# kch3782/torcwa

Measured on AMD Instinct MI355X. Metric: RCWA layer-solves/sec (complex64 I/O) at Fourier order [15,15], higher is better.
Workload: dtype c128 results (mixed-precision eigensolver: fp32 eigendecomposition refined to fp64 by two Newton steps -- fp64 residual and update GEMMs, the correction solved with ONE fp32 LU of the fp32 start; everything else fp64 MFMA); complex64 I/O; 1 GPU; configs[1]: single patterned layer, order=[15,15] (n=1922), 300x300 grid, 128-lambda sweep, glass input half-space; points_total=128, points_per_gpu=128, layer_solves_per_point=1, chunk=128, streams=1, precision=high

## Files before the change

torcwa_amd/csrc/eig_qr.hip:

```cpp
#include "eig.hpp"
#include <cstdlib>
#include <limits>
#include <mutex>
#include <string>
#include <thread>
#include <vector>
#include "mfma.hpp"
#include "prof.hpp"

namespace trx {
namespace {

constexpr int QW = EigPlan::QW, QNS = EigPlan::QNS, QKC = EigPlan::QKC;
constexpr int SM = 64;
constexpr int QAED = EigPlan::QAED;
constexpr int QAED_MOVES = 12;

template <class T>
struct Rot {
    T c;
    cx<T> s, r;
};

template <class T>
// ... 31 lines not shown
        if (!(big < std::numeric_limits<T>::infinity())) { R.c = T(1); R.s = cx<T>(T(0), T(0)); R.r = f; return R; }
        int ex;
        (void)frexp((double)big, &ex);
        const T sc = (T)ldexp(1.0, -ex), isc = (T)ldexp(1.0, ex);
        const cx<T> fs = sc * f, gs = sc * g;
        const T a2 = norm2(fs), g2 = norm2(gs), m2 = a2 + g2;
        if (a2 == T(0)) { const T ng = sqrt(g2); R.c = T(0); R.s = (T(1) / ng) * conj(gs); R.r = cx<T>(ng * isc, T(0)); return R; }
        const T t2 = T(1) / sqrt(a2 * m2);
        R.c = a2 * t2;
        R.s = t2 * (fs * conj(gs));
        R.r = ((m2 * t2) * isc) * fs;
    }
    return R;
}

template <class T, bool BC = false>
__device__ bool small_schur(cx<T>* Hs, int m, cx<T>* Us, Rot<T>* rots, const int SLD, long long* dbg = nullptr, int* nrot_out = nullptr) {
    const auto sync = [] { __syncthreads(); };
    const int lane = threadIdx.x;
    long long t_left = 0, t_right = 0, t_u = 0, t_pre = 0, tt = 0, n_it = 0, n_rot = 0;
    if (dbg) tt = clock64();
    const T ulp = eps_of<T>::value;
    int ihi = m - 1, its = 0, total = 0, nrot = 0;
    while (ihi > 0) {
        int small = 0;
        if (lane >= 1 && lane <= ihi) {
            const cx<T> sub = Hs[lane * SLD + lane - 1];
            T sc = abs1(Hs[(lane - 1) * SLD + lane - 1]) + abs1(Hs[lane * SLD + lane]);
            if (sc == T(0)) sc = T(1);
            small = (abs1(sub) <= ulp * sc);
            if (small) Hs[lane * SLD + lane - 1] = cx<T>(T(0), T(0));
        }
        const unsigned long long mask = __ballot(small);
        const int l = mask ? (63 - __builtin_clzll(mask)) : 0;
        sync();
        if (l == ihi) { --ihi; its = 0; continue; }
        ++its; ++total;
        if (total > 40 * m) { if (nrot_out) *nrot_out = nrot; return false; }
        nrot += ihi - l;
        cx<T> sig;
        {
            const cx<T> a = Hs[(ihi - 1) * SLD + ihi - 1], bq = Hs[(ihi - 1) * SLD + ihi], cq = Hs[ihi * SLD + ihi - 1], d = Hs[ihi * SLD + ihi];
            if (its % 10 == 0) {
                sig = d + cx<T>(T(0.75) * fabs(cq.x), T(0));
            } else {
                const cx<T> tr = T(0.5) * (a + d);
                const cx<T> det = (a - tr) * (d - tr) - bq * cq;
                const cx<T> sq = csqrt(-det);
                const cx<T> e1 = tr + sq, e2 = tr - sq;
                sig = (abs1(e1 - d) < abs1(e2 - d)) ? e1 : e2;
            }
        }
        sync();
        if (lane >= l && lane <= ihi) Hs[lane * SLD + lane] -= sig;
        sync();
        if (dbg) { const long long t1 = clock64(); t_pre += t1 - tt; tt = t1; n_it += 1; n_rot += ihi - l; }
        {
            const bool mine = (lane >= l && lane < m);
            cx<T> xcur = mine ? Hs[l * SLD + lane] : cx<T>(T(0), T(0));
            cx<T> ynext = (mine && l + 1 <= ihi) ? Hs[(l + 1) * SLD + lane] : cx<T>(T(0), T(0));
            for (int r = l; r < ihi; ++r) {
                const cx<T> ypre = (mine && r + 2 <= ihi) ? Hs[(r + 2) * SLD + lane] : cx<T>(T(0), T(0));
                Rot<T> R;
                if constexpr (BC) {
                    R = rotg_fast(bcast_lane(xcur, r), bcast_lane(ynext, r));
                } else {
                    R.c = T(1); R.s = cx<T>(T(0), T(0)); R.r = cx<T>(T(0), T(0));
                    if (lane == r) R = rotg_fast(xcur, ynext);
                    R.c = __shfl(R.c, r);
                    R.s.x = __shfl(R.s.x, r); R.s.y = __shfl(R.s.y, r);
                    R.r.x = __shfl(R.r.x, r); R.r.y = __shfl(R.r.y, r);
                }
                if (lane == r) rots[r] = R;
                if (lane >= r && lane < m) {
                    cx<T> x = xcur, y = ynext;
                    rot_rows(R, x, y);
                    if (lane == r) { x = R.r; y = cx<T>(T(0), T(0)); Hs[(r + 1) * SLD + lane] = y; }
                    Hs[r * SLD + lane] = x;
                    xcur = y;
                }
                ynext = ypre;
            }
            if (lane >= ihi && lane < m) Hs[ihi * SLD + lane] = xcur;
        }
        sync();
        if (dbg) { const long long t1 = clock64(); t_left += t1 - tt; tt = t1; }
        {
        if (lane <= ihi) {
            const int i = lane;
            const int r0 = (i - 1 > l) ? i - 1 : l;
            if (r0 < ihi) {
                cx<T> x = Hs[i * SLD + r0];
                for (int r = r0; r < ihi; ++r) {
                    cx<T> y = Hs[i * SLD + r + 1];
                    rot_cols(rots[r], x, y);
                    Hs[i * SLD + r] = x;
                    x = y;
                }
                Hs[i * SLD + ihi] = x;
            }
        }
        if (dbg) { sync(); const long long t1 = clock64(); t_right += t1 - tt; tt = t1; }
        if (Us && lane < m && l < ihi) {
            cx<T> x = Us[lane * SLD + l];
            for (int r = l; r < ihi; ++r) {
                cx<T> y = Us[lane * SLD + r + 1];
                rot_cols(rots[r], x, y);
                Us[lane * SLD + r] = x;
                x = y;
            }
            Us[lane * SLD + ihi] = x;
        }
        sync();
        if (dbg) { const long long t1 = clock64(); t_u += t1 - tt; tt = t1; }
        }
        if (lane >= l && lane <= ihi) Hs[lane * SLD + lane] += sig;
        sync();
    }
    if (dbg && lane == 0) { dbg[0] += t_pre; dbg[1] += t_left; dbg[2] += t_right; dbg[3] += t_u; dbg[4] += n_it; dbg[5] += n_rot; }
    if (nrot_out) *nrot_out = nrot;
    return true;
}

template <class T>
__device__ void schur_swap(cx<T>* Ts, cx<T>* Vs, int m, int k, const int SLD) {
    const auto sync = [] { __syncthreads(); };
    const int lane = threadIdx.x;
    const cx<T> a = Ts[k * SLD + k], bq = Ts[(k + 1) * SLD + k + 1], x = Ts[k * SLD + k + 1];
    const Rot<T> R = rotg_fast(x, bq - a);
    sync();
    if (lane >= k && lane < m) {
        cx<T> u = Ts[k * SLD + lane], v = Ts[(k + 1) * SLD + lane];
        rot_rows(R, u, v);
        Ts[k * SLD + lane] = u; Ts[(k + 1) * SLD + lane] = v;
    }
    if (lane < m) {
        cx<T> u = Vs[lane * SLD + k], v = Vs[lane * SLD + k + 1];
        rot_cols(R, u, v);
        Vs[lane * SLD + k] = u; Vs[lane * SLD + k + 1] = v;
    }
    sync();
    if (lane <= k + 1) {
        cx<T> u = Ts[lane * SLD + k], v = Ts[lane * SLD + k + 1];
        rot_cols(R, u, v);
        if (lane == k + 1) u = cx<T>(T(0), T(0));
        Ts[lane * SLD + k] = u; Ts[lane * SLD + k + 1] = v;
    }
    sync();
}

template <class T>
__device__ void small_larfg(const cx<T>* x, int inc, int len, cx<T>* vw, cx<T>& tau, T& beta) {
    const auto sync = [] { __syncthreads(); };
    const int lane = threadIdx.x;
    const cx<T> alpha = x[0];
    T xn2 = (lane >= 1 && lane < len) ? norm2(x[lane * inc]) : T(0);
    xn2 = wave_sum(xn2);
    cx<T> scale;
    if (xn2 == T(0) && alpha.y == T(0)) {
        tau = cx<T>(T(0), T(0)); beta = alpha.x; scale = cx<T>(T(0), T(0));
    } else {
        const T nrm = sqrt(norm2(alpha) + xn2);
        beta = (alpha.x >= T(0)) ? -nrm : nrm;
        tau = cx<T>((beta - alpha.x) / beta, -alpha.y / beta);
        scale = crecip(cx<T>(alpha.x - beta, alpha.y));
    }
    sync();
    if (lane < len) vw[lane] = (lane == 0) ? cx<T>(T(1), T(0)) : x[lane * inc] * scale;
    sync();
}

template <class T>
__device__ void small_apply_reflector(cx<T>* Ts, cx<T>* Vs, int m, int nrows_t, int o, int len, int c0, const cx<T>* vw, cx<T> tau, const int SLD) {
    const auto sync = [] { __syncthreads(); };
    const int lane = threadIdx.x;
    if (lane >= c0 && lane < m) {
        cx<T> w(T(0), T(0));
        for (int i = 0; i < len; ++i) cfma_conj(w, vw[i], Ts[(o + i) * SLD + lane]);
        const cx<T> f = conj(tau) * w;
        for (int i = 0; i < len; ++i) Ts[(o + i) * SLD + lane] -= vw[i] * f;
    }
    sync();
    if (lane < nrows_t) {
        cx<T> w(T(0), T(0));
        for (int i = 0; i < len; ++i) cfma(w, Ts[lane * SLD + o + i], vw[i]);
        const cx<T> f = tau * w;
        for (int i = 0; i < len; ++i) Ts[lane * SLD + o + i] -= f * conj(vw[i]);
    }
    if (lane < m) {
        cx<T> w(T(0), T(0));
        for (int i = 0; i < len; ++i) cfma(w, Vs[lane * SLD + o + i], vw[i]);
        const cx<T> f = tau * w;
        for (int i = 0; i < len; ++i) Vs[lane * SLD + o + i] -= f * conj(vw[i]);
    }
    sync();
}

template <class T>
__global__ __launch_bounds__(64) void qr_init_kernel(QrState* __restrict__ st, int n) {
    if (threadIdx.x == 0) {
        QrState s;
        s.ilo = 0; s.ihi = n - 1; s.nch = 0; s.mode = QR_IDLE; s.stall = 0; s.sweeps = 0; s.fail = 0;
        for (int c = 0; c < QKC; ++c) { s.k[c] = 0; s.tau[c][0] = s.tau[c][1] = 1; s.tau_last[c] = 0; s.w0[c] = 0; s.w1[c] = 0; }
        st[blockIdx.x] = s;
    }
}

__device__ __forceinline__ void clear_windows(QrState& st) {
// ... 8 lines not shown
    int ktot = avail < QNS * room ? avail : QNS * room;
    if (ktot < 0) ktot = 0;
    st.nch = (ktot + QNS - 1) / QNS;
#pragma unroll
    for (int c = 0; c < QKC; ++c) {
        int kc = ktot - QNS * c;
        kc = kc < 0 ? 0 : (kc > QNS ? QNS : kc);
        st.k[c] = kc;
        if (kc > 0) { st.tau[c][0] = st.tau[c][1] = 0; st.tau_last[c] = (ihi - 1 - ilo) + 2 * (kc - 1); }
        else { st.tau[c][0] = st.tau[c][1] = 1; st.tau_last[c] = 0; }
    }
    return ktot;
}
__device__ __forceinline__ int chain_shift_pos(const QrState& st, int ktot, int c, int s) { return ktot - QNS * c - st.k[c] + s; }

template <class T, bool BC>
__global__ __launch_bounds__(64) void qr_prepare_kernel(cx<T>* __restrict__ Aall, long mstride, int n, QrState* __restrict__ stall_,
                                                        cx<T>* __restrict__ Uall, cx<T>* __restrict__ shifts_all,
                                                        int* __restrict__ summary, int max_sweeps, int aed_w, int nibble, int aed_moves, int par, int max_chains,
                                                        int sm, int* __restrict__ counters, long long* dbg_all = nullptr) {
    TRX_DYN_SMEM(smem);
    long long* dbg = (dbg_all && blockIdx.x == 0) ? dbg_all : nullptr;
    long long tk0 = dbg ? clock64() : 0;
    const int SLD = sm + 1;
    const int QNMIN = sm;
    cx<T>* Hs = reinterpret_cast<cx<T>*>(smem);
    cx<T>* Us = Hs + sm * SLD;
    cx<T>* vwork = Us + sm * SLD;
    cx<T>* wk = vwork + sm;
    Rot<T>* rots = reinterpret_cast<Rot<T>*>(wk + sm);
    QrState& sst = *reinterpret_cast<QrState*>(rots + sm);
    const int b = blockIdx.x, lane = threadIdx.x;
    cx<T>* H = Aall + (long)b * mstride;
    if (lane == 0) sst = stall_[b];
    __syncthreads();
    QrState st = sst;
    if (st.mode == QR_DONE) return;
    if (st.mode == QR_CHASE) {
        bool unfinished = false;
        for (int c = 0; c < st.nch; ++c) unfinished = unfinished || (st.tau[c][par] <= st.tau_last[c]);
        if (unfinished) {
            if (lane == 0) { atomicAdd(&summary[0], 1); atomicOr(&summary[2], 2); atomicMax(&summary[1], st.ihi + 1); }
            return;
        }
    }
    const T ulp = eps_of<T>::value;
    int bad = 0;
    for (int i = 1 + lane; i <= st.ihi; i += 64) {
        const cx<T> sub = H[(long)i * n + i - 1];
        const cx<T> dg = H[(long)i * n + i];
        if (!(abs1(sub) + abs1(dg) < std::numeric_limits<T>::infinity())) bad = 1;
        if (sub.x != T(0) || sub.y != T(0)) {
            T s = abs1(H[(long)(i - 1) * n + i - 1]) + abs1(H[(long)i * n + i]);
            if (s == T(0)) s = T(1);
            if (abs1(sub) <= ulp * s) H[(long)i * n + i - 1] = cx<T>(T(0), T(0));
        }
    }
    __syncthreads();
    if (__any(bad)) {
        if (lane == 0) { st.fail += st.ihi + 1; st.mode = QR_DONE; clear_windows(st); stall_[b] = st; }
        return;
    }
    int ihi = 0;
    for (int base = st.ihi; base >= 1; base -= 64) {
        const int i = base - lane;
        int pred = 0;
        if (i >= 1) { const cx<T> sub = H[(long)i * n + i - 1]; pred = (sub.x != T(0) || sub.y != T(0)); }
        const unsigned long long mask = __ballot(pred);
        if (mask) { ihi = base - __builtin_ctzll(mask); break; }
    }
    if (ihi <= 0) {
        if (lane == 0) { st.ihi = 0; st.mode = QR_DONE; clear_windows(st); stall_[b] = st; }
        return;
    }
    int ilo = 0;
    for (int base = ihi - 1; base >= 1; base -= 64) {
        const int i = base - lane;
        int pred = 0;
        if (i >= 1) { const cx<T> sub = H[(long)i * n + i - 1]; pred = (sub.x == T(0) && sub.y == T(0)); }
        const unsigned long long mask = __ballot(pred);
        if (mask) { ilo = base - __builtin_ctzll(mask); break; }
    }
    if (ihi != st.ihi || ilo != st.ilo) st.stall = 0;
    st.ihi = ihi; st.ilo = ilo;
    const int m = ihi - ilo + 1;
    if (m <= QNMIN) {
        for (int e = lane; e < m * m; e += 64) {
            const int r = e / m, c = e - r * m;
            Hs[r * SLD + c] = (r <= c + 1) ? H[(long)(ilo + r) * n + ilo + c] : cx<T>(T(0), T(0));
            Us[r * SLD + c] = cx<T>(r == c ? T(1) : T(0), T(0));
        }
        __syncthreads();
        int nrot = 0;
        const bool ok = small_schur<T, BC>(Hs, m, Us, rots, SLD, nullptr, &nrot);
        if (lane == 0) atomicAdd(&counters[1], nrot);
        __syncthreads();
        cx<T>* U = Uall + (long)b * QW * QW;
        for (int e = lane; e < m * m; e += 64) {
            const int r = e / m, c = e - r * m;
            H[(long)(ilo + r) * n + ilo + c] = (r <= c) ? Hs[r * SLD + c] : cx<T>(T(0), T(0));
            U[r * QW + c] = Us[r * SLD + c];
        }
        if (lane == 0) {
            clear_windows(st);
            st.w0[0] = ilo; st.w1[0] = ihi + 1;
            st.mode = QR_SMALL_PENDING; st.ihi = ilo - 1; st.ilo = 0; st.stall = 0;
            if (!ok) st.fail += m;
            stall_[b] = st;
            atomicAdd(&summary[0], 1);
            atomicOr(&summary[2], 1);
            atomicMax(&summary[1], st.ihi + 1);
        }
        return;
    }
    if (st.sweeps >= max_sweeps) {
        if (lane == 0) { st.fail += ihi + 1; st.mode = QR_DONE; clear_windows(st); stall_[b] = st; }
        return;
    }
    const int nw = aed_w;
    const int kw = ihi - nw + 1;
    cx<T> spike = H[(long)kw * n + kw - 1];
    for (int e = lane; e < nw * nw; e += 64) {
        const int r = e / nw, c = e - r * nw;
        Hs[r * SLD + c] = (r <= c + 1) ? H[(long)(kw + r) * n + kw + c] : cx<T>(T(0), T(0));
        Us[r * SLD + c] = cx<T>(r == c ? T(1) : T(0), T(0));
    }
    __syncthreads();
    if (dbg && lane == 0) { const long long t1 = clock64(); dbg[6] += t1 - tk0; tk0 = t1; }
    int nrot = 0;
    const bool okw = small_schur<T, BC>(Hs, nw, Us, rots, SLD, dbg, &nrot);
    if (lane == 0) atomicAdd(&counters[1], nrot);
    __syncthreads();
    if (dbg && lane == 0) { const long long t1 = clock64(); dbg[7] += t1 - tk0; tk0 = t1; }
    int ns = nw;
    if (okw) {
        const T smlnum = eps_of<T>::safmin * ((T)n / ulp);
        int ilst = 0, moves = 0;
        while (ilst < ns) {
            T foo = abs1(Hs[(ns - 1) * SLD + ns - 1]);
            if (foo == T(0)) foo = abs1(spike);
            const T sp = abs1(spike) * abs1(Us[ns - 1]);
            const T thr = (smlnum > ulp * foo) ? smlnum : ulp * foo;
            if (sp <= thr) {
                --ns;
            } else {
                if (moves >= aed_moves) break;
                for (int kk = ns - 2; kk >= ilst; --kk) schur_swap<T>(Hs, Us, nw, kk, SLD);
                ++ilst; ++moves;
            }
        }
    }
    const int nd = nw - ns;
    if (dbg && lane == 0) { const long long t1 = clock64(); dbg[8] += t1 - tk0; tk0 = t1; dbg[11] += 1; }
    cx<T>* sh = shifts_all + (long)b * QKC * QNS;
    if (nd == 0) {
        int avail = m / 2 < nw ? m / 2 : nw;
        const int k = plan_chains(st, ilo, ihi, avail, max_chains);
        {
            const int c = lane / QNS, sidx = lane - c * QNS;
            if (c < st.nch && sidx < st.k[c]) {
                const int pos = nw - k + chain_shift_pos(st, k, c, sidx);
                cx<T> sv = Hs[pos * SLD + pos];
                if (st.stall > 0 && (st.stall % 6) == 0) {
                    const T mag = T(0.75) * cabs(H[(long)ihi * n + ihi - 1]);
                    const T ang = T(6.283185307179586) * (T)lane / (T)k;
                    sv = sv + cx<T>(mag * (T)cos(ang), mag * (T)sin(ang));
                }
                sh[c * QNS + sidx] = sv;
            }
        }
        if (lane == 0) {
            st.mode = QR_CHASE;
            st.stall += 1; st.sweeps += 1; clear_windows(st);
            stall_[b] = st;
            atomicAdd(&summary[0], 1);
            atomicMax(&summary[1], ihi + 1);
        }
        return;
    }
    if (ns == 0) spike = cx<T>(T(0), T(0));
    const int m2 = (ihi - nd) - ilo + 1;
    int kch = 0;
    QrState stc = st;
    if (nd * 100 < nibble * nw && m2 > QNMIN && ns >= 2) {
        kch = plan_chains(stc, ilo, ihi - nd, (m2 / 2 < ns) ? m2 / 2 : ns, max_chains);
        const int c = lane / QNS, sidx = lane - c * QNS;
        if (kch >= 2 && c < stc.nch && sidx < stc.k[c]) {
            const int pos = ns - kch + chain_shift_pos(stc, kch, c, sidx);
            sh[c * QNS + sidx] = Hs[pos * SLD + pos];
        }
    }
    if (ns > 1 && (spike.x != T(0) || spike.y != T(0))) {
        cx<T>* vw = vwork;
        if (lane < ns) wk[lane] = conj(Us[lane]);
        __syncthreads();
        cx<T> tau; T beta;
        small_larfg<T>(wk, 1, ns, vw, tau, beta);
        small_apply_reflector<T>(Hs, Us, nw, ns, 0, ns, 0, vw, tau, SLD);
        for (int jc = 0; jc + 2 < ns; ++jc) {
            small_larfg<T>(Hs + (jc + 1) * SLD + jc, SLD, ns - jc - 1, vw, tau, beta);
            if (lane == 0) Hs[(jc + 1) * SLD + jc] = cx<T>(beta, T(0));
            if (lane >= 1 && lane < ns - jc - 1) Hs[(jc + 1 + lane) * SLD + jc] = cx<T>(T(0), T(0));
            __syncthreads();
            small_apply_reflector<T>(Hs, Us, nw, ns, jc + 1, ns - jc - 1, jc + 1, vw, tau, SLD);
        }
    }
    __syncthreads();
    if (dbg && lane == 0) { const long long t1 = clock64(); dbg[9] += t1 - tk0; tk0 = t1; }
    {
        cx<T>* U = Uall + (long)b * QW * QW;
        for (int e = lane; e < nw * nw; e += 64) {
            const int r = e / nw, c = e - r * nw;
            cx<T> v = Hs[r * SLD + c];
            if (r > c + 1 || (r == c + 1 && r >= ns)) v = cx<T>(T(0), T(0));
            H[(long)(kw + r) * n + kw + c] = v;
            U[r * QW + c] = Us[r * SLD + c];
        }
        if (lane == 0) {
            H[(long)kw * n + kw - 1] = spike * conj(Us[0]);
            if (kch >= 2) {
                const int sw = st.sweeps;
                st = stc;
                st.mode = QR_AED_CHASE;
                st.ihi = ihi - nd;
                st.sweeps = sw + 1;
                atomicMax(&summary[1], st.ihi + 1);
            } else {
                st.mode = QR_SMALL_PENDING;
            }
            clear_windows(st);
            st.w0[0] = kw; st.w1[0] = ihi + 1; st.stall = 0;
            stall_[b] = st;
            atomicAdd(&summary[0], 1);
// ... 858 lines not shown
}

template <class T>
__global__ void qr_collect_info_kernel(const QrState* __restrict__ st, int* __restrict__ info, int batch, int ngroups) {
    const int b = blockIdx.x * blockDim.x + threadIdx.x;
    if (b >= batch) return;
    const int g = b % ngroups, local = b / ngroups;
    int b0 = 0;
    for (int h = 0; h < g; ++h) b0 += (batch - h + ngroups - 1) / ngroups;
    info[b] = st[b0 + local].fail;
}

}

struct QrKnobs {
    int groups = 0, spw = 0, aed = 0, nibble = 100, moves = QAED_MOVES, chains = 0, band = 0, rotb = 0, super = 0, defer = 0, fuse = 0;
    bool debug = false;
};
static QrKnobs& qr_knobs() {
    static QrKnobs k = [] {
        QrKnobs q;
        auto geti = [](const char* name, int lo, int hi, int dflt) {
            const char* e = getenv(name);
            if (!e) return dflt;
            const int v = atoi(e);
            return (v >= lo && v <= hi) ? v : dflt;
        };
        q.groups = geti("TRX_QR_GROUPS", 1, 8, 0);
        q.spw = geti("TRX_SLAB_SPW", 1, 4, 0);
        if (q.spw == 3) q.spw = 0;
        q.aed = geti("TRX_QR_AED", 16, QAED, 0);
        q.nibble = geti("TRX_QR_NIBBLE", 0, 100, 100);
        q.moves = geti("TRX_QR_MOVES", 0, QAED, QAED_MOVES);
        q.chains = geti("TRX_QR_CHAINS", 1, QKC, 0);
        q.band = geti("TRX_SLAB_BAND", 0, 2, 0);
        q.rotb = geti("TRX_QR_ROTB", 0, 1, 0);
        q.super = geti("TRX_QR_SUPER", 1, QSUPER, 0);
        q.defer = geti("TRX_QR_DEFER", 0, 2, 0);
        q.fuse = geti("TRX_QR_FUSE", 0, 2, 0);
        q.debug = getenv("TRX_QR_DEBUG") != nullptr;
        return q;
    }();
    return k;
}

int qr_chains_for(int batch) { const QrKnobs& K = qr_knobs(); return K.chains ? K.chains : (batch <= 2 ? QKC : (batch <= 48 ? 2 : 1)); }
int qr_log_slots(int n) { return cdiv_i(n + 2 * QNS, QW - 2 * QNS - 1) + 2 + 4 * (QKC - 1) + 1; }

struct QrLane {
    hipStream_t s = nullptr;
    hipEvent_t ev = nullptr;
// ... 22 lines not shown
static void lane_return(const QrLane& l) {
    std::lock_guard<std::mutex> lock(g_lane_mu);
    g_lane_free.push_back(l);
}

int qr_set_knob(const char* key, int value) {
    QrKnobs& k = qr_knobs();
    const std::string s(key);
    int* slot = nullptr;
    int lo = 0, hi = 0;
    if (s == "qr_groups") { slot = &k.groups; hi = 8; }
    else if (s == "slab_spw") { slot = &k.spw; hi = 4; }
    else if (s == "qr_aed") { slot = &k.aed; hi = QAED; }
    else if (s == "qr_nibble") { slot = &k.nibble; hi = 100; }
    else if (s == "qr_moves") { slot = &k.moves; hi = QAED; }
    else if (s == "qr_rotb") { slot = &k.rotb; hi = 1; }
    else if (s == "qr_chains") { slot = &k.chains; hi = QKC; }
    else if (s == "slab_band") { slot = &k.band; hi = 2; }
    else if (s == "qr_super") { slot = &k.super; hi = QSUPER; }
    else if (s == "qr_defer") { slot = &k.defer; hi = 2; }
    else if (s == "qr_fuse") { slot = &k.fuse; hi = 2; }
    else return TRX_ERR_ARG;
    if (value < lo || value > hi || (slot == &k.spw && value == 3) || (slot == &k.aed && value != 0 && value < 16)) return TRX_ERR_ARG;
    *slot = value;
    return TRX_OK;
}

template <class T>
int hessenberg_qr(hipStream_t s, const EigBuffers<T>& B, int n, int batch, int* info) {
    constexpr int LD = QW + 1;
    if ((double)n * n * sizeof(cx<T>) >= 4294967296.0) return TRX_ERR_ARG;
    const QrKnobs& K = qr_knobs();
    const size_t smw = sizeof(cx<T>) * QW * LD + sizeof(RotCS<T>) * WMAXS * QNS + sizeof(QrState) + 16;
    const int kc = qr_chains_for(batch);
    const int nslot = qr_log_slots(n);
    const size_t sma = sizeof(T) * 2 * QW * MLD + 16 + sizeof(QrLink) * (size_t)nslot * kc;
    auto smp_of = [](int sm) { return sizeof(cx<T>) * (2 * (size_t)sm * (sm + 1) + 2 * sm) + sizeof(Rot<T>) * sm + sizeof(QrState); };
    static std::mutex attr_mu;
    static int attr_state[64][2];
    int attr_rc = 0, dev_attr = 0;
    (void)hipGetDevice(&dev_attr);
    {
        std::lock_guard<std::mutex> lock(attr_mu);
        int& stt = attr_state[dev_attr & 63][sizeof(T) == 8];
        if (stt == 0) {
            const size_t sma_max = 160 * 1024 - 512;
            const int r = set_max_dyn_smem((const void*)qr_window_kernel<T, false>, smw) || set_max_dyn_smem((const void*)qr_window_kernel<T, true>, smw) ||
                  set_max_dyn_smem((const void*)apply_links_kernel<T, 0>, sma_max) || set_max_dyn_smem((const void*)apply_links_kernel<T, 1>, sma_max) ||
                  set_max_dyn_smem((const void*)apply_links_kernel<T, 2>, sma_max) ||
                  set_max_dyn_smem((const void*)qr_prepare_kernel<T, false>, smp_of(SM)) || set_max_dyn_smem((const void*)qr_prepare_kernel<T, true>, smp_of(SM));
            stt = r ? 2 : 1;
        }
        attr_rc = stt == 2;
    }
    if (attr_rc) return TRX_ERR_LAUNCH;
    TRX_LAUNCH((qr_init_kernel<T>), dim3(batch), dim3(64), 0, s, B.st, n);
    if (hipMemsetAsync(B.summary, 0, sizeof(int) * 128, s) != hipSuccess) return TRX_ERR_LAUNCH;
    const int max_sweeps = 30 * n + 100;
    const int spw = K.spw ? K.spw : 1;
    const int nstrip = cdiv_i(n, 16);
    const int adv = QW - 2 * QNS - 1;
    const int band_on = K.band != 1;
    const int super = kc == 1 ? (K.super ? K.super : (sizeof(T) == 4 ? 4 : 8)) : 1;
    const bool defer = kc == 1 && K.defer != 1;
    const bool fuse = defer && K.fuse != 1;
// ... 40 lines not shown
        if (!lane_checkout(dev, g > 0, G.lane)) { rc = TRX_ERR_LAUNCH; break; }
        ++nlanes;
        G.s = g == 0 ? s : G.lane.s;
        if (g > 0 && hipStreamWaitEvent(G.s, fork.ev, 0) != hipSuccess) { rc = TRX_ERR_LAUNCH; break; }
    }
    const long mstride = (long)ngroups * n * n;
    const int aed_w = K.aed ? K.aed : ((batch >= 64 || kc >= 2) ? QAED : 48);
    const size_t smp = smp_of(aed_w);
    const int nibble = K.nibble, aed_moves = K.moves;
    const bool qr_debug = K.debug;
    long long* dbg_dev = reinterpret_cast<long long*>(B.summary + 128);
    auto issue_prepare = [&](Group& G, int slot) -> bool {
        int* sum = G.summary + 4 * slot;
        if (hipMemsetAsync(sum, 0, sizeof(int) * 3, G.s) != hipSuccess) return false;
        { ProfScope prof(PROF_QR_PREPARE, G.s, 0, 0);
          if (K.rotb == 1)
              TRX_LAUNCH((qr_prepare_kernel<T, false>), dim3(G.nb), dim3(64), smp, G.s, B.A + (long)G.g * n * n, mstride, n, B.st + G.b0, B.U + (long)G.b0 * QW * QW,
                         B.shifts + (long)G.b0 * QKC * QNS, sum, max_sweeps, aed_w, nibble, aed_moves, G.par, kc, aed_w, G.summary + 8,
                         (qr_debug && G.b0 == 0) ? dbg_dev : (long long*)nullptr);
          else
              TRX_LAUNCH((qr_prepare_kernel<T, true>), dim3(G.nb), dim3(64), smp, G.s, B.A + (long)G.g * n * n, mstride, n, B.st + G.b0, B.U + (long)G.b0 * QW * QW,
                         B.shifts + (long)G.b0 * QKC * QNS, sum, max_sweeps, aed_w, nibble, aed_moves, G.par, kc, aed_w, G.summary + 8,
                         (qr_debug && G.b0 == 0) ? dbg_dev : (long long*)nullptr); }
        if (hipMemcpyAsync(G.lane.hsum + 4 * slot, sum, sizeof(int) * 3, hipMemcpyDeviceToHost, G.s) != hipSuccess) return false;
        return hipEventRecord(G.lane.evs[slot], G.s) == hipSuccess;
    };
    auto issue_sweep = [&](Group& G, int bound) -> bool {
        cx<T>* Ag = B.A + (long)G.g * n * n;
        cx<T>* Zg = B.Z + (long)G.g * n * n;
        const cx<T>* Ud = B.U + (long)G.b0 * QW * QW;
        cx<T>* Ul = B.Ulog + (long)G.b0 * nslot * kc * QW * QW;
        QrLink* lk = B.links + (long)G.b0 * nslot * kc;
        const cx<T>* shg = B.shifts + (long)G.b0 * QKC * QNS;
        QrState* stg = B.st + G.b0;
        int nwin = bound > 0 ? cdiv_i(bound + 2 * QNS, adv) + 2 + 4 * (kc - 1) : 1;
        if (nwin > nslot) nwin = nslot;
// ... 92 lines not shown
            for (int i = 0; i < 5; ++i) work[i] += G.work[i];
        }
        if (g > 0) {
            if (hipEventRecord(G.lane.ev, G.s) != hipSuccess || hipStreamWaitEvent(s, G.lane.ev, 0) != hipSuccess) rc = rc ? rc : TRX_ERR_LAUNCH;
            if (hipStreamSynchronize(G.s) != hipSuccess) rc = rc ? rc : TRX_ERR_LAUNCH;
        } else if (G.issued > 0) {
            if (hipEventSynchronize(G.lane.evs[(G.issued - 1) & 1]) != hipSuccess) rc = rc ? rc : TRX_ERR_LAUNCH;
        }
        lane_return(G.lane);
    }
    if (ngroups > 1) lane_return(fork);
    if (rc) return rc;
    if (qr_debug) {
        long long h[24];
        if (hipMemcpyAsync(h, dbg_dev, sizeof(h), hipMemcpyDeviceToHost, s) == hipSuccess && hipStreamSynchronize(s) == hipSuccess)
            fprintf(stderr, "libtrx qr_prepare cycles (matrix 0, %lld AED calls): scan+load %lld | schur %lld (pre %lld left %lld right %lld U %lld; %lld iterations, %lld rotations) | "
                            "reorder %lld | restore %lld | store %lld || window kernel: load %lld chase %lld (%lld chain steps) store %lld; per phase: rotg %lld left %lld barrier %lld right %lld barrier %lld\n",
                    h[11], h[6], h[7], h[0], h[1], h[2], h[3], h[4], h[5], h[8], h[9], h[10], h[12], h[13], h[15], h[14], h[16], h[17], h[18], h[19], h[20]);
    }
    if (prof_enabled()) {
        prof_add_work(PROF_QR_APPLY_LEFT, 8.0 * 4096.0 * work[0], 2.0 * sizeof(cx<T>) * 4096.0 * work[0] / QW);
        prof_add_work(PROF_QR_APPLY_RIGHT, 8.0 * 4096.0 * work[1], 2.0 * sizeof(cx<T>) * 4096.0 * work[1] / QW);
        prof_add_work(PROF_QR_WINDOW, work[2] / batch, 8.0 * 4096.0 * work[4]);
        prof_add_work(PROF_QR_PREPARE, work[3] / batch, 0.0);
    }
    TRX_LAUNCH((qr_collect_info_kernel<T>), dim3(cdiv_i(batch, 64)), dim3(64), 0, s, (const QrState*)B.st, info, batch, ngroups);
    TRX_CHECK_LAUNCH();
    return TRX_OK;
}

template int hessenberg_qr<float>(hipStream_t, const EigBuffers<float>&, int, int, int*);
// ... 4 lines not shown
```

Before: 37.81 layer-solves/s.

## Pipeline AED small Schur across four waves with blocked right rotations

The AED prepare kernel goes from one wave to four. In small_schur, wave 0 computes the Givens rotations for the left sweep in blocks of eight while three helper waves apply the rotations of earlier blocks to H columns and to U, and the shift subtraction is folded into the rotation passes. Reflector application and schur_swap also split their row and column updates across waves. This aims to cut the serial latency of the single-wave AED QR, at the cost of more barriers, a larger block and changed shift-timing semantics (its+1), which could alter convergence.

```diff
diff --git a/torcwa_amd/csrc/eig_qr.hip b/torcwa_amd/csrc/eig_qr.hip
--- a/torcwa_amd/csrc/eig_qr.hip
+++ b/torcwa_amd/csrc/eig_qr.hip
@@ -69,110 +69,116 @@
     return R;
 }
 
-template <class T, bool BC = false>
-__device__ bool small_schur(cx<T>* Hs, int m, cx<T>* Us, Rot<T>* rots, const int SLD, long long* dbg = nullptr, int* nrot_out = nullptr) {
+constexpr int PWAVES = 4, PTHREADS = 64 * PWAVES;
+constexpr int RBLK = 8;
+
+template <class T>
+__device__ bool small_schur(cx<T>* Hs, int m, cx<T>* Us, Rot<T>* rots, cx<T>* xch, const int SLD, long long* dbg = nullptr, int* nrot_out = nullptr) {
     const auto sync = [] { __syncthreads(); };
-    const int lane = threadIdx.x;
-    long long t_left = 0, t_right = 0, t_u = 0, t_pre = 0, tt = 0, n_it = 0, n_rot = 0;
+    const int tid = threadIdx.x, lane = tid & 63, wave = tid >> 6;
+    long long t_left = 0, t_right = 0, t_help = 0, t_pre = 0, tt = 0, n_it = 0, n_rot = 0;
     if (dbg) tt = clock64();
     const T ulp = eps_of<T>::value;
     int ihi = m - 1, its = 0, total = 0, nrot = 0;
     while (ihi > 0) {
-        int small = 0;
-        if (lane >= 1 && lane <= ihi) {
-            const cx<T> sub = Hs[lane * SLD + lane - 1];
-            T sc = abs1(Hs[(lane - 1) * SLD + lane - 1]) + abs1(Hs[lane * SLD + lane]);
-            if (sc == T(0)) sc = T(1);
-            small = (abs1(sub) <= ulp * sc);
-            if (small) Hs[lane * SLD + lane - 1] = cx<T>(T(0), T(0));
-        }
-        const unsigned long long mask = __ballot(small);
-        const int l = mask ? (63 - __builtin_clzll(mask)) : 0;
+        if (wave == 0) {
+            int small = 0;
+            if (lane >= 1 && lane <= ihi) {
+                const cx<T> sub = Hs[lane * SLD + lane - 1];
+                T sc = abs1(Hs[(lane - 1) * SLD + lane - 1]) + abs1(Hs[lane * SLD + lane]);
+                if (sc == T(0)) sc = T(1);
+                small = (abs1(sub) <= ulp * sc);
+                if (small) Hs[lane * SLD + lane - 1] = cx<T>(T(0), T(0));
+            }
+            const unsigned long long mask = __ballot(small);
+            const int lw = mask ? (63 - __builtin_clzll(mask)) : 0;
+            cx<T> sg(T(0), T(0));
+            if (lw < ihi) {
+                const cx<T> a = Hs[(ihi - 1) * SLD + ihi - 1], bq = Hs[(ihi - 1) * SLD + ihi], cq = Hs[ihi * SLD + ihi - 1], d = Hs[ihi * SLD + ihi];
+                if ((its + 1) % 10 == 0) {
+                    sg = d + cx<T>(T(0.75) * fabs(cq.x), T(0));
+                } else {
+                    const cx<T> tr = T(0.5) * (a + d);
+                    const cx<T> det = (a - tr) * (d - tr) - bq * cq;
+                    const cx<T> sq = csqrt(-det);
+                    const cx<T> e1 = tr + sq, e2 = tr - sq;
+                    sg = (abs1(e1 - d) < abs1(e2 - d)) ? e1 : e2;
+                }
+            }
+            if (lane == 0) { xch[0] = cx<T>((T)lw, T(0)); xch[1] = sg; }
+        }
+        sync();
+        const int l = (int)xch[0].x;
+        const cx<T> sig = xch[1];
         sync();
         if (l == ihi) { --ihi; its = 0; continue; }
         ++its; ++total;
         if (total > 40 * m) { if (nrot_out) *nrot_out = nrot; return false; }
         nrot += ihi - l;
-        cx<T> sig;
-        {
-            const cx<T> a = Hs[(ihi - 1) * SLD + ihi - 1], bq = Hs[(ihi - 1) * SLD + ihi], cq = Hs[ihi * SLD + ihi - 1], d = Hs[ihi * SLD + ihi];
-            if (its % 10 == 0) {
-                sig = d + cx<T>(T(0.75) * fabs(cq.x), T(0));
+        if (dbg) { const long long t1 = clock64(); t_pre += t1 - tt; tt = t1; n_it += 1; n_rot += ihi - l; }
+        const int nb = (ihi - l + RBLK - 1) / RBLK;
+        const bool mine = (lane >= l && lane < m);
+        cx<T> xcur(T(0), T(0)), ynext(T(0), T(0));
+        if (wave == 0 && mine) {
+            xcur = Hs[l * SLD + lane];
+            if (lane == l) xcur -= sig;
+            if (l + 1 <= ihi) { ynext = Hs[(l + 1) * SLD + lane]; if (lane == l + 1) ynext -= sig; }
+        }
+        int rdone = l;
+        for (int j = 0; j <= nb; ++j) {
+            if (wave == 0) {
+                if (j < nb) {
+                    const int r1 = (l + (j + 1) * RBLK < ihi) ? l + (j + 1) * RBLK : ihi;
+                    for (int r = l + j * RBLK; r < r1; ++r) {
+                        cx<T> ypre(T(0), T(0));
+                        if (mine && r + 2 <= ihi) { ypre = Hs[(r + 2) * SLD + lane]; if (lane == r + 2) ypre -= sig; }
+                        const Rot<T> R = rotg_fast(bcast_lane(xcur, r), bcast_lane(ynext, r));
+                        if (lane == r) rots[r] = R;
+                        if (lane >= r && lane < m) {
+                            cx<T> x = xcur, y = ynext;
+                            rot_rows(R, x, y);
+                            if (lane == r) { x = R.r; y = cx<T>(T(0), T(0)); Hs[(r + 1) * SLD + lane] = y; }
+                            Hs[r * SLD + lane] = x;
+                            xcur = y;
+                        }
+                        ynext = ypre;
+                    }
+                    if (r1 == ihi && lane >= ihi && lane < m) Hs[ihi * SLD + lane] = xcur;
+                }
             } else {
-                const cx<T> tr = T(0.5) * (a + d);
-                const cx<T> det = (a - tr) * (d - tr) - bq * cq;
-                const cx<T> sq = csqrt(-det);
-                const cx<T> e1 = tr + sq, e2 = tr - sq;
-                sig = (abs1(e1 - d) < abs1(e2 - d)) ? e1 : e2;
-            }
-        }
-        sync();
-        if (lane >= l && lane <= ihi) Hs[lane * SLD + lane] -= sig;
-        sync();
-        if (dbg) { const long long t1 = clock64(); t_pre += t1 - tt; tt = t1; n_it += 1; n_rot += ihi - l; }
-        {
-            const bool mine = (lane >= l && lane < m);
-            cx<T> xcur = mine ? Hs[l * SLD + lane] : cx<T>(T(0), T(0));
-            cx<T> ynext = (mine && l + 1 <= ihi) ? Hs[(l + 1) * SLD + lane] : cx<T>(T(0), T(0));
-            for (int r = l; r < ihi; ++r) {
-                const cx<T> ypre = (mine && r + 2 <= ihi) ? Hs[(r + 2) * SLD + lane] : cx<T>(T(0), T(0));
-                Rot<T> R;
-                if constexpr (BC) {
-                    R = rotg_fast(bcast_lane(xcur, r), bcast_lane(ynext, r));
-                } else {
-                    R.c = T(1); R.s = cx<T>(T(0), T(0)); R.r = cx<T>(T(0), T(0));
-                    if (lane == r) R = rotg_fast(xcur, ynext);
-                    R.c = __shfl(R.c, r);
-                    R.s.x = __shfl(R.s.x, r); R.s.y = __shfl(R.s.y, r);
-                    R.r.x = __shfl(R.r.x, r); R.r.y = __shfl(R.r.y, r);
+                const long long th = (dbg && tid == 64) ? clock64() : 0;
+                const int rhi = j < nb ? l + j * RBLK - 1 : ihi;
+                if (rhi > rdone) {
+                    const int nh = ihi + 1, ntask = nh + (Us ? m : 0);
+                    for (int t = tid - 64; t < ntask; t += PTHREADS - 64) {
+                        const bool onh = t < nh;
+                        cx<T>* X = onh ? Hs : Us;
+                        const int i = onh ? t : t - nh;
+                        int r0 = rdone;
+                        if (onh && i - 1 > r0) r0 = i - 1;
+                        if (r0 >= rhi) continue;
+                        cx<T> x = X[i * SLD + r0];
+                        for (int r = r0; r < rhi; ++r) {
+                            cx<T> y = X[i * SLD + r + 1];
+                            rot_cols(rots[r], x, y);
+                            if (onh && r == i) x += sig;
+                            X[i * SLD + r] = x;
+                            x = y;
+                        }
+                        if (onh && rhi == ihi && i == ihi) x += sig;
+                        X[i * SLD + rhi] = x;
+                    }
+                    rdone = rhi;
                 }
-                if (lane == r) rots[r] = R;
-                if (lane >= r && lane < m) {
-                    cx<T> x = xcur, y = ynext;
-                    rot_rows(R, x, y);
-                    if (lane == r) { x = R.r; y = cx<T>(T(0), T(0)); Hs[(r + 1) * SLD + lane] = y; }
-                    Hs[r * SLD + lane] = x;
-                    xcur = y;
-                }
-                ynext = ypre;
-            }
-            if (lane >= ihi && lane < m) Hs[ihi * SLD + lane] = xcur;
-        }
-        sync();
-        if (dbg) { const long long t1 = clock64(); t_left += t1 - tt; tt = t1; }
-        {
-        if (lane <= ihi) {
-            const int i = lane;
-            const int r0 = (i - 1 > l) ? i - 1 : l;
-            if (r0 < ihi) {
-                cx<T> x = Hs[i * SLD + r0];
-                for (int r = r0; r < ihi; ++r) {
-                    cx<T> y = Hs[i * SLD + r + 1];
-                    rot_cols(rots[r], x, y);
-                    Hs[i * SLD + r] = x;
-                    x = y;
-                }
-                Hs[i * SLD + ihi] = x;
-            }
-        }
-        if (dbg) { sync(); const long long t1 = clock64(); t_right += t1 - tt; tt = t1; }
-        if (Us && lane < m && l < ihi) {
-            cx<T> x = Us[lane * SLD + l];
-            for (int r = l; r < ihi; ++r) {
-                cx<T> y = Us[lane * SLD + r + 1];
-                rot_cols(rots[r], x, y);
-                Us[lane * SLD + r] = x;
-                x = y;
-            }
-            Us[lane * SLD + ihi] = x;
-        }
-        sync();
-        if (dbg) { const long long t1 = clock64(); t_u += t1 - tt; tt = t1; }
-        }
-        if (lane >= l && lane <= ihi) Hs[lane * SLD + lane] += sig;
-        sync();
-    }
-    if (dbg && lane == 0) { dbg[0] += t_pre; dbg[1] += t_left; dbg[2] += t_right; dbg[3] += t_u; dbg[4] += n_it; dbg[5] += n_rot; }
+                if (dbg && tid == 64) t_help += clock64() - th;
+            }
+            sync();
+            if (dbg && tid == 0 && j == nb - 1) { const long long t1 = clock64(); t_left += t1 - tt; tt = t1; }
+        }
+        if (dbg && tid == 0) { const long long t1 = clock64(); t_right += t1 - tt; tt = t1; }
+    }
+    if (dbg && tid == 0) { dbg[0] += t_pre; dbg[1] += t_left; dbg[2] += t_right; dbg[4] += n_it; dbg[5] += n_rot; }
+    if (dbg && tid == 64) dbg[3] += t_help;
     if (nrot_out) *nrot_out = nrot;
     return true;
 }
@@ -180,34 +186,35 @@
 template <class T>
 __device__ void schur_swap(cx<T>* Ts, cx<T>* Vs, int m, int k, const int SLD) {
     const auto sync = [] { __syncthreads(); };
-    const int lane = threadIdx.x;
+    const int tid = threadIdx.x, lane = tid & 63, wave = tid >> 6;
     const cx<T> a = Ts[k * SLD + k], bq = Ts[(k + 1) * SLD + k + 1], x = Ts[k * SLD + k + 1];
     const Rot<T> R = rotg_fast(x, bq - a);
     sync();
-    if (lane >= k && lane < m) {
-        cx<T> u = Ts[k * SLD + lane], v = Ts[(k + 1) * SLD + lane];
-        rot_rows(R, u, v);
-        Ts[k * SLD + lane] = u; Ts[(k + 1) * SLD + lane] = v;
-    }
-    if (lane < m) {
+    if (wave == 0) {
+        if (lane >= k && lane < m) {
+            cx<T> u = Ts[k * SLD + lane], v = Ts[(k + 1) * SLD + lane];
+            rot_rows(R, u, v);
+            Ts[k * SLD + lane] = u; Ts[(k + 1) * SLD + lane] = v;
+        }
+        wave_sync();
+        if (lane <= k + 1) {
+            cx<T> u = Ts[lane * SLD + k], v = Ts[lane * SLD + k + 1];
+            rot_cols(R, u, v);
+            if (lane == k + 1) u = cx<T>(T(0), T(0));
+            Ts[lane * SLD + k] = u; Ts[lane * SLD + k + 1] = v;
+        }
+    } else if (wave == 1 && lane < m) {
         cx<T> u = Vs[lane * SLD + k], v = Vs[lane * SLD + k + 1];
         rot_cols(R, u, v);
         Vs[lane * SLD + k] = u; Vs[lane * SLD + k + 1] = v;
     }
     sync();
-    if (lane <= k + 1) {
-        cx<T> u = Ts[lane * SLD + k], v = Ts[lane * SLD + k + 1];
-        rot_cols(R, u, v);
-        if (lane == k + 1) u = cx<T>(T(0), T(0));
-        Ts[lane * SLD + k] = u; Ts[lane * SLD + k + 1] = v;
-    }
-    sync();
 }
 
 template <class T>
 __device__ void small_larfg(const cx<T>* x, int inc, int len, cx<T>* vw, cx<T>& tau, T& beta) {
     const auto sync = [] { __syncthreads(); };
-    const int lane = threadIdx.x;
+    const int tid = threadIdx.x, lane = tid & 63;
     const cx<T> alpha = x[0];
     T xn2 = (lane >= 1 && lane < len) ? norm2(x[lane * inc]) : T(0);
     xn2 = wave_sum(xn2);
@@ -221,32 +228,36 @@
         scale = crecip(cx<T>(alpha.x - beta, alpha.y));
     }
     sync();
-    if (lane < len) vw[lane] = (lane == 0) ? cx<T>(T(1), T(0)) : x[lane * inc] * scale;
+    if (tid < len) vw[tid] = (tid == 0) ? cx<T>(T(1), T(0)) : x[tid * inc] * scale;
     sync();
 }
 
 template <class T>
 __device__ void small_apply_reflector(cx<T>* Ts, cx<T>* Vs, int m, int nrows_t, int o, int len, int c0, const cx<T>* vw, cx<T> tau, const int SLD) {
     const auto sync = [] { __syncthreads(); };
-    const int lane = threadIdx.x;
-    if (lane >= c0 && lane < m) {
-        cx<T> w(T(0), T(0));
-        for (int i = 0; i < len; ++i) cfma_conj(w, vw[i], Ts[(o + i) * SLD + lane]);
-        const cx<T> f = conj(tau) * w;
-        for (int i = 0; i < len; ++i) Ts[(o + i) * SLD + lane] -= vw[i] * f;
-    }
-    sync();
-    if (lane < nrows_t) {
-        cx<T> w(T(0), T(0));
-        for (int i = 0; i < len; ++i) cfma(w, Ts[lane * SLD + o + i], vw[i]);
-        const cx<T> f = tau * w;
-        for (int i = 0; i < len; ++i) Ts[lane * SLD + o + i] -= f * conj(vw[i]);
-    }
-    if (lane < m) {
+    const int tid = threadIdx.x, lane = tid & 63, wave = tid >> 6;
+    if (wave == 0) {
+        if (lane >= c0 && lane < m) {
+            cx<T> w(T(0), T(0));
+            for (int i = 0; i < len; ++i) cfma_conj(w, vw[i], Ts[(o + i) * SLD + lane]);
+            const cx<T> f = conj(tau) * w;
+            for (int i = 0; i < len; ++i) Ts[(o + i) * SLD + lane] -= vw[i] * f;
+        }
+    } else if (wave == 1 && lane < m) {
         cx<T> w(T(0), T(0));
         for (int i = 0; i < len; ++i) cfma(w, Vs[lane * SLD + o + i], vw[i]);
         const cx<T> f = tau * w;
         for (int i = 0; i < len; ++i) Vs[lane * SLD + o + i] -= f * conj(vw[i]);
+    }
+    sync();
+    {
+        const int row = 2 * lane + (wave & 1);
+        if (wave >= 2 && row < nrows_t) {
+            cx<T> w(T(0), T(0));
+            for (int i = 0; i < len; ++i) cfma(w, Ts[row * SLD + o + i], vw[i]);
+            const cx<T> f = tau * w;
+            for (int i = 0; i < len; ++i) Ts[row * SLD + o + i] -= f * conj(vw[i]);
+        }
     }
     sync();
 }
@@ -285,8 +296,8 @@
 }
 __device__ __forceinline__ int chain_shift_pos(const QrState& st, int ktot, int c, int s) { return ktot - QNS * c - st.k[c] + s; }
 
-template <class T, bool BC>
-__global__ __launch_bounds__(64) void qr_prepare_kernel(cx<T>* __restrict__ Aall, long mstride, int n, QrState* __restrict__ stall_,
+template <class T>
+__global__ __launch_bounds__(PTHREADS) void qr_prepare_kernel(cx<T>* __restrict__ Aall, long mstride, int n, QrState* __restrict__ stall_,
                                                         cx<T>* __restrict__ Uall, cx<T>* __restrict__ shifts_all,
                                                         int* __restrict__ summary, int max_sweeps, int aed_w, int nibble, int aed_moves, int par, int max_chains,
                                                         int sm, int* __restrict__ counters, long long* dbg_all = nullptr) {
@@ -300,10 +311,12 @@
     cx<T>* vwork = Us + sm * SLD;
     cx<T>* wk = vwork + sm;
     Rot<T>* rots = reinterpret_cast<Rot<T>*>(wk + sm);
-    QrState& sst = *reinterpret_cast<QrState*>(rots + sm);
-    const int b = blockIdx.x, lane = threadIdx.x;
+    cx<T>* xch = reinterpret_cast<cx<T>*>(rots + sm);
+    QrState& sst = *reinterpret_cast<QrState*>(xch + 2);
+    int& sbad = *reinterpret_cast<int*>(xch);
+    const int b = blockIdx.x, tid = threadIdx.x, lane = tid & 63, wave = tid >> 6;
     cx<T>* H = Aall + (long)b * mstride;
-    if (lane == 0) sst = stall_[b];
+    if (tid == 0) { sst = stall_[b]; sbad = 0; }
     __syncthreads();
     QrState st = sst;
     if (st.mode == QR_DONE) return;
@@ -311,13 +324,13 @@
         bool unfinished = false;
         for (int c = 0; c < st.nch; ++c) unfinished = unfinished || (st.tau[c][par] <= st.tau_last[c]);
         if (unfinished) {
-            if (lane == 0) { atomicAdd(&summary[0], 1); atomicOr(&summary[2], 2); atomicMax(&summary[1], st.ihi + 1); }
+            if (tid == 0) { atomicAdd(&summary[0], 1); atomicOr(&summary[2], 2); atomicMax(&summary[1], st.ihi + 1); }
             return;
         }
     }
     const T ulp = eps_of<T>::value;
     int bad = 0;
-    for (int i = 1 + lane; i <= st.ihi; i += 64) {
+    for (int i = 1 + tid; i <= st.ihi; i += PTHREADS) {
         const cx<T> sub = H[(long)i * n + i - 1];
         const cx<T> dg = H[(long)i * n + i];
         if (!(abs1(sub) + abs1(dg) < std::numeric_limits<T>::infinity())) bad = 1;
@@ -327,9 +340,10 @@
             if (abs1(sub) <= ulp * s) H[(long)i * n + i - 1] = cx<T>(T(0), T(0));
         }
     }
+    if (__any(bad) && lane == 0) atomicOr(&sbad, 1);
     __syncthreads();
-    if (__any(bad)) {
-        if (lane == 0) { st.fail += st.ihi + 1; st.mode = QR_DONE; clear_windows(st); stall_[b] = st; }
+    if (sbad) {
+        if (tid == 0) { st.fail += st.ihi + 1; st.mode = QR_DONE; clear_windows(st); stall_[b] = st; }
         return;
     }
     int ihi = 0;
@@ -341,7 +355,7 @@
         if (mask) { ihi = base - __builtin_ctzll(mask); break; }
     }
     if (ihi <= 0) {
-        if (lane == 0) { st.ihi = 0; st.mode = QR_DONE; clear_windows(st); stall_[b] = st; }
+        if (tid == 0) { st.ihi = 0; st.mode = QR_DONE; clear_windows(st); stall_[b] = st; }
         return;
     }
     int ilo = 0;
@@ -356,23 +370,23 @@
     st.ihi = ihi; st.ilo = ilo;
     const int m = ihi - ilo + 1;
     if (m <= QNMIN) {
-        for (int e = lane; e < m * m; e += 64) {
+        for (int e = tid; e < m * m; e += PTHREADS) {
             const int r = e / m, c = e - r * m;
             Hs[r * SLD + c] = (r <= c + 1) ? H[(long)(ilo + r) * n + ilo + c] : cx<T>(T(0), T(0));
             Us[r * SLD + c] = cx<T>(r == c ? T(1) : T(0), T(0));
         }
         __syncthreads();
         int nrot = 0;
-        const bool ok = small_schur<T, BC>(Hs, m, Us, rots, SLD, nullptr, &nrot);
-        if (lane == 0) atomicAdd(&counters[1], nrot);
+        const bool ok = small_schur<T>(Hs, m, Us, rots, xch, SLD, nullptr, &nrot);
+        if (tid == 0) atomicAdd(&counters[1], nrot);
         __syncthreads();
         cx<T>* U = Uall + (long)b * QW * QW;
-        for (int e = lane; e < m * m; e += 64) {
+        for (int e = tid; e < m * m; e += PTHREADS) {
             const int r = e / m, c = e - r * m;
             H[(long)(ilo + r) * n + ilo + c] = (r <= c) ? Hs[r * SLD + c] : cx<T>(T(0), T(0));
             U[r * QW + c] = Us[r * SLD + c];
         }
-        if (lane == 0) {
+        if (tid == 0) {
             clear_windows(st);
             st.w0[0] = ilo; st.w1[0] = ihi + 1;
             st.mode = QR_SMALL_PENDING; st.ihi = ilo - 1; st.ilo = 0; st.stall = 0;
@@ -385,24 +399,24 @@
         return;
     }
     if (st.sweeps >= max_sweeps) {
-        if (lane == 0) { st.fail += ihi + 1; st.mode = QR_DONE; clear_windows(st); stall_[b] = st; }
+        if (tid == 0) { st.fail += ihi + 1; st.mode = QR_DONE; clear_windows(st); stall_[b] = st; }
         return;
     }
     const int nw = aed_w;
     const int kw = ihi - nw + 1;
     cx<T> spike = H[(long)kw * n + kw - 1];
-    for (int e = lane; e < nw * nw; e += 64) {
+    for (int e = tid; e < nw * nw; e += PTHREADS) {
         const int r = e / nw, c = e - r * nw;
         Hs[r * SLD + c] = (r <= c + 1) ? H[(long)(kw + r) * n + kw + c] : cx<T>(T(0), T(0));
         Us[r * SLD + c] = cx<T>(r == c ? T(1) : T(0), T(0));
     }
     __syncthreads();
-    if (dbg && lane == 0) { const long long t1 = clock64(); dbg[6] += t1 - tk0; tk0 = t1; }
+    if (dbg && tid == 0) { const long long t1 = clock64(); dbg[6] += t1 - tk0; tk0 = t1; }
     int nrot = 0;
-    const bool okw = small_schur<T, BC>(Hs, nw, Us, rots, SLD, dbg, &nrot);
-    if (lane == 0) atomicAdd(&counters[1], nrot);
+    const bool okw = small_schur<T>(Hs, nw, Us, rots, xch, SLD, dbg, &nrot);
+    if (tid == 0) atomicAdd(&counters[1], nrot);
     __syncthreads();
-    if (dbg && lane == 0) { const long long t1 = clock64(); dbg[7] += t1 - tk0; tk0 = t1; }
+    if (dbg && tid == 0) { const long long t1 = clock64(); dbg[7] += t1 - tk0; tk0 = t1; }
     int ns = nw;
     if (okw) {
         const T smlnum = eps_of<T>::safmin * ((T)n / ulp);
@@ -422,12 +436,12 @@
         }
     }
     const int nd = nw - ns;
-    if (dbg && lane == 0) { const long long t1 = clock64(); dbg[8] += t1 - tk0; tk0 = t1; dbg[11] += 1; }
+    if (dbg && tid == 0) { const long long t1 = clock64(); dbg[8] += t1 - tk0; tk0 = t1; dbg[11] += 1; }
     cx<T>* sh = shifts_all + (long)b * QKC * QNS;
     if (nd == 0) {
         int avail = m / 2 < nw ? m / 2 : nw;
         const int k = plan_chains(st, ilo, ihi, avail, max_chains);
-        {
+        if (wave == 0) {
             const int c = lane / QNS, sidx = lane - c * QNS;
             if (c < st.nch && sidx < st.k[c]) {
                 const int pos = nw - k + chain_shift_pos(st, k, c, sidx);
@@ -440,7 +454,7 @@
                 sh[c * QNS + sidx] = sv;
             }
         }
-        if (lane == 0) {
+        if (tid == 0) {
             st.mode = QR_CHASE;
             st.stall += 1; st.sweeps += 1; clear_windows(st);
             stall_[b] = st;
@@ -456,38 +470,38 @@
     if (nd * 100 < nibble * nw && m2 > QNMIN && ns >= 2) {
         kch = plan_chains(stc, ilo, ihi - nd, (m2 / 2 < ns) ? m2 / 2 : ns, max_chains);
         const int c = lane / QNS, sidx = lane - c * QNS;
-        if (kch >= 2 && c < stc.nch && sidx < stc.k[c]) {
+        if (wave == 0 && kch >= 2 && c < stc.nch && sidx < stc.k[c]) {
             const int pos = ns - kch + chain_shift_pos(stc, kch, c, sidx);
             sh[c * QNS + sidx] = Hs[pos * SLD + pos];
         }
     }
     if (ns > 1 && (spike.x != T(0) || spike.y != T(0))) {
         cx<T>* vw = vwork;
-        if (lane < ns) wk[lane] = conj(Us[lane]);
+        if (tid < ns) wk[tid] = conj(Us[tid]);
         __syncthreads();
         cx<T> tau; T beta;
         small_larfg<T>(wk, 1, ns, vw, tau, beta);
         small_apply_reflector<T>(Hs, Us, nw, ns, 0, ns, 0, vw, tau, SLD);
         for (int jc = 0; jc + 2 < ns; ++jc) {
             small_larfg<T>(Hs + (jc + 1) * SLD + jc, SLD, ns - jc - 1, vw, tau, beta);
-            if (lane == 0) Hs[(jc + 1) * SLD + jc] = cx<T>(beta, T(0));
-            if (lane >= 1 && lane < ns - jc - 1) Hs[(jc + 1 + lane) * SLD + jc] = cx<T>(T(0), T(0));
+            if (tid == 0) Hs[(jc + 1) * SLD + jc] = cx<T>(beta, T(0));
+            if (tid >= 1 && tid < ns - jc - 1) Hs[(jc + 1 + tid) * SLD + jc] = cx<T>(T(0), T(0));
             __syncthreads();
             small_apply_reflector<T>(Hs, Us, nw, ns, jc + 1, ns - jc - 1, jc + 1, vw, tau, SLD);
         }
     }
     __syncthreads();
-    if (dbg && lane == 0) { const long long t1 = clock64(); dbg[9] += t1 - tk0; tk0 = t1; }
+    if (dbg && tid == 0) { const long long t1 = clock64(); dbg[9] += t1 - tk0; tk0 = t1; }
     {
         cx<T>* U = Uall + (long)b * QW * QW;
-        for (int e = lane; e < nw * nw; e += 64) {
+        for (int e = tid; e < nw * nw; e += PTHREADS) {
             const int r = e / nw, c = e - r * nw;
             cx<T> v = Hs[r * SLD + c];
             if (r > c + 1 || (r == c + 1 && r >= ns)) v = cx<T>(T(0), T(0));
             H[(long)(kw + r) * n + kw + c] = v;
             U[r * QW + c] = Us[r * SLD + c];
         }
-        if (lane == 0) {
+        if (tid == 0) {
             H[(long)kw * n + kw - 1] = spike * conj(Us[0]);
             if (kch >= 2) {
                 const int sw = st.sweeps;
@@ -1376,7 +1390,7 @@
 }
 
 struct QrKnobs {
-    int groups = 0, spw = 0, aed = 0, nibble = 100, moves = QAED_MOVES, chains = 0, band = 0, rotb = 0, super = 0, defer = 0, fuse = 0;
+    int groups = 0, spw = 0, aed = 0, nibble = 100, moves = QAED_MOVES, chains = 0, band = 0, super = 0, defer = 0, fuse = 0;
     bool debug = false;
 };
 static QrKnobs& qr_knobs() {
@@ -1396,7 +1410,6 @@
         q.moves = geti("TRX_QR_MOVES", 0, QAED, QAED_MOVES);
         q.chains = geti("TRX_QR_CHAINS", 1, QKC, 0);
         q.band = geti("TRX_SLAB_BAND", 0, 2, 0);
-        q.rotb = geti("TRX_QR_ROTB", 0, 1, 0);
         q.super = geti("TRX_QR_SUPER", 1, QSUPER, 0);
         q.defer = geti("TRX_QR_DEFER", 0, 2, 0);
         q.fuse = geti("TRX_QR_FUSE", 0, 2, 0);
@@ -1449,7 +1462,6 @@
     else if (s == "qr_aed") { slot = &k.aed; hi = QAED; }
     else if (s == "qr_nibble") { slot = &k.nibble; hi = 100; }
     else if (s == "qr_moves") { slot = &k.moves; hi = QAED; }
-    else if (s == "qr_rotb") { slot = &k.rotb; hi = 1; }
     else if (s == "qr_chains") { slot = &k.chains; hi = QKC; }
     else if (s == "slab_band") { slot = &k.band; hi = 2; }
     else if (s == "qr_super") { slot = &k.super; hi = QSUPER; }
@@ -1470,7 +1482,7 @@
     const int kc = qr_chains_for(batch);
     const int nslot = qr_log_slots(n);
     const size_t sma = sizeof(T) * 2 * QW * MLD + 16 + sizeof(QrLink) * (size_t)nslot * kc;
-    auto smp_of = [](int sm) { return sizeof(cx<T>) * (2 * (size_t)sm * (sm + 1) + 2 * sm) + sizeof(Rot<T>) * sm + sizeof(QrState); };
+    auto smp_of = [](int sm) { return sizeof(cx<T>) * (2 * (size_t)sm * (sm + 1) + 2 * sm + 2) + sizeof(Rot<T>) * sm + sizeof(QrState); };
     static std::mutex attr_mu;
     static int attr_state[64][2];
     int attr_rc = 0, dev_attr = 0;
@@ -1483,7 +1495,7 @@
             const int r = set_max_dyn_smem((const void*)qr_window_kernel<T, false>, smw) || set_max_dyn_smem((const void*)qr_window_kernel<T, true>, smw) ||
                   set_max_dyn_smem((const void*)apply_links_kernel<T, 0>, sma_max) || set_max_dyn_smem((const void*)apply_links_kernel<T, 1>, sma_max) ||
                   set_max_dyn_smem((const void*)apply_links_kernel<T, 2>, sma_max) ||
-                  set_max_dyn_smem((const void*)qr_prepare_kernel<T, false>, smp_of(SM)) || set_max_dyn_smem((const void*)qr_prepare_kernel<T, true>, smp_of(SM));
+                  set_max_dyn_smem((const void*)qr_prepare_kernel<T>, smp_of(SM));
             stt = r ? 2 : 1;
         }
         attr_rc = stt == 2;
@@ -1554,12 +1566,7 @@
         int* sum = G.summary + 4 * slot;
         if (hipMemsetAsync(sum, 0, sizeof(int) * 3, G.s) != hipSuccess) return false;
         { ProfScope prof(PROF_QR_PREPARE, G.s, 0, 0);
-          if (K.rotb == 1)
-              TRX_LAUNCH((qr_prepare_kernel<T, false>), dim3(G.nb), dim3(64), smp, G.s, B.A + (long)G.g * n * n, mstride, n, B.st + G.b0, B.U + (long)G.b0 * QW * QW,
-                         B.shifts + (long)G.b0 * QKC * QNS, sum, max_sweeps, aed_w, nibble, aed_moves, G.par, kc, aed_w, G.summary + 8,
-                         (qr_debug && G.b0 == 0) ? dbg_dev : (long long*)nullptr);
-          else
-              TRX_LAUNCH((qr_prepare_kernel<T, true>), dim3(G.nb), dim3(64), smp, G.s, B.A + (long)G.g * n * n, mstride, n, B.st + G.b0, B.U + (long)G.b0 * QW * QW,
+          TRX_LAUNCH((qr_prepare_kernel<T>), dim3(G.nb), dim3(PTHREADS), smp, G.s, B.A + (long)G.g * n * n, mstride, n, B.st + G.b0, B.U + (long)G.b0 * QW * QW,
                          B.shifts + (long)G.b0 * QKC * QNS, sum, max_sweeps, aed_w, nibble, aed_moves, G.par, kc, aed_w, G.summary + 8,
                          (qr_debug && G.b0 == 0) ? dbg_dev : (long long*)nullptr); }
         if (hipMemcpyAsync(G.lane.hsum + 4 * slot, sum, sizeof(int) * 3, hipMemcpyDeviceToHost, G.s) != hipSuccess) return false;
@@ -1682,7 +1689,7 @@
     if (qr_debug) {
         long long h[24];
         if (hipMemcpyAsync(h, dbg_dev, sizeof(h), hipMemcpyDeviceToHost, s) == hipSuccess && hipStreamSynchronize(s) == hipSuccess)
-            fprintf(stderr, "libtrx qr_prepare cycles (matrix 0, %lld AED calls): scan+load %lld | schur %lld (pre %lld left %lld right %lld U %lld; %lld iterations, %lld rotations) | "
+            fprintf(stderr, "libtrx qr_prepare cycles (matrix 0, %lld AED calls): scan+load %lld | schur %lld (pre %lld left %lld right tail %lld, helper waves busy %lld; %lld iterations, %lld rotations) | "
                             "reorder %lld | restore %lld | store %lld || window kernel: load %lld chase %lld (%lld chain steps) store %lld; per phase: rotg %lld left %lld barrier %lld right %lld barrier %lld\n",
                     h[11], h[6], h[7], h[0], h[1], h[2], h[3], h[4], h[5], h[8], h[9], h[10], h[12], h[13], h[15], h[14], h[16], h[17], h[18], h[19], h[20]);
     }
```

New measurement: 38.17 layer-solves/s (median of 6 runs). No clear change (+0.9%).
